# elchemista/vettore

Measured on AMD Instinct MI355X. Metric: queries/sec, flat cosine top-10, N=10000000 d=768 (achieved HBM GB/s in roofline), higher is better.
Workload: dtype f32; 1 GPU; index: :flat, metric: :cosine, d=768, N=10000000, limit=10, single query in flight; rows_per_gpu=10000000, reduce_order=sse2, processes=1

## Files before the change

vettore_amd/csrc/host/vt_search.h:

```cpp
#pragma once

namespace {

enum : unsigned { NEED_RANKS = 1, NEED_STRICT_RANKS = 2, NEED_BITS = 4, NEED_NORMS = 8, NEED_NZBITS = 16, NEED_SKETCH = 32 };
constexpr int kEscalate = -101;

bool lazy_ranks_ok(const Shard *ix, size_t limit) {
  const size_t lazy_want = std::min<size_t>(limit, ix->n) + (limit < ix->n ? 1 : 0);
  const size_t kmax = vt::scan_lds_bytes((uint32_t)ix->dim, vt::kMaxFusedK) ? (size_t)vt::kMaxFusedK : (size_t)vt::kSmallK;
  return !ix->ranks_clean && !ix->external_ranks && lazy_want <= kmax &&
         ix->unranked <= std::max<size_t>(65536, ix->n / 8);
}

constexpr size_t kPatternMinRows = 16384, kPatternMaxWant = 8 * (size_t)vt::kMaxFusedK;
bool pattern_metric(int metric) {
  return metric == VT_HAMMING || metric == VT_JACCARD;
}
bool pattern_search_applies(const Shard *ix, size_t limit) {
  return pattern_metric(ix->metric) && !ix->nz_bits.refused && ix->n >= kPatternMinRows &&
         std::min<size_t>(limit, ix->n) + 1 <= kPatternMaxWant;
}

bool shadow_metric(int metric) {
  return metric == VT_COSINE || metric == VT_INNER_PRODUCT || metric == VT_NEG_INNER_PRODUCT || metric == VT_L2 ||
// ... 269 lines not shown
  VT_HIP(vt::launch_sketch_tail(ta, c.stream));
  VT_HIP(hipStreamSynchronize(c.stream));
  if (c.hSkInfo.p[0] == 2u) {
    VT_TRY(c.ensure_part_lists((size_t)kSketchRescoreBlocks * k));
    vt::ScanArgs sa = scan_args(ix, c, d);
    set_gather(sa, gather_of(c.dSkRows.p), kSketchCandCap);
    sa.k = k;
    use_part_lists(sa, c);
    sa.batch_counts = c.dSkCount.p;
    sa.batch_cap = kSketchCandCap;
    VT_HIP(vt::launch_scan_batch(sa, kSketchRescoreBlocks, 1, c.stream));
    VT_HIP(vt::launch_select(c.dPartKeys.p, c.dPartPay.p, kSketchRescoreBlocks * k, k, 0, 0, c.dStatus.p, c.dResMapped,
                             c.dSelKeys.p, c.dSelPay.p, c.stream));
    VT_HIP(hipStreamSynchronize(c.stream));
  }
  const bool certified = c.hSkInfo.p[0] != 0u && c.hRes.p->status == 0;
  if (c.profiling) {
    float ms = 0.f;
    VT_TRY(c.span_ms(&ms));
    const uint64_t bytes = (uint64_t)vt::sketch_bytes(ix->n, d);
    c.prof.sketch_launches += 1;
    c.prof.sketch_ms += ms;
    c.prof.sketch_bytes += bytes;
    c.prof.sketch_candidates += c.hSkInfo.p[1];
    c.prof.sketch_tail_rescored += c.hSkInfo.p[0] == 1u ? 1 : 0;
    VT_TRY(c.book_scan(1, ix->n, bytes));
  }
  if (!certified) {
    c.prof.sketch_fallbacks += 1;
    return VT_OK;
  }
  std::vector<vt::Entry> entries(c.hRes.p->e, c.hRes.p->e + c.hRes.p->count);
  VT_TRY(make_hits(ix, entries, out));
  *done = true;
  return VT_OK;
}

int sketch6_search(Shard *ix, Ctx &c, const float *query, size_t limit, bool *done, vt_hits **out, int bits = 6) {
  const SketchKind &kind = sketch_kind(bits);
  const bool five = bits == 5;
  *done = false;
  const uint32_t d = (uint32_t)ix->dim, ld = ix->ld, ld8 = vt::sketch_ld8(d);
  double qq = 0.0;
  for (uint32_t i = 0; i < d; ++i) qq += (double)query[i] * (double)query[i];
  const double up = 1.0 + 0x1p-30;
  const double qn = std::sqrt(qq) * up;
  if (!(qn * ix->*kind.max_norm * up < 0x1p126)) return VT_OK;
  const uint32_t lw = vt_host::sketch6_level_words(d);
  const size_t qwords = (size_t)ld + (size_t)vt::kSketch6Levels * lw;
  const size_t chain_zeros = vt::kScanFilterSyncWords;
  const size_t total = qwords + (kind.exact_threshold ? chain_zeros : 0);
  VT_TRY(c.dQ.ensure(total));
  VT_TRY(c.hQ.ensure(total));
  if (c.hSkResid.size() < d) c.hSkResid.resize(d);
  float *hq = c.hQ.p;
  std::memcpy(hq, query, (size_t)d * sizeof(float));
  for (uint32_t i = d; i < ld; ++i) hq[i] = 0.0f;
  float t[vt::kSketch6Levels];
  double ee = 0.0;
  static_assert(vt::kSketch6Levels == vt_host::kSketch6Levels, "one number of query levels on both sides");
  vt_host::sketch6_query_levels(query, d, reinterpret_cast<uint32_t *>(hq + ld), c.hSkResid.data(), t, &ee);
  if (kind.exact_threshold) std::memset(hq + qwords, 0, chain_zeros * sizeof(float));
  uint32_t *chain_words = reinterpret_cast<uint32_t *>(c.dQ.p + qwords);
  c.qbits_kind = 0;
  c.qsrc = c.dQ.p;
  VT_HIP(hipMemcpyAsync(c.dQ.p, c.hQ.p, total * sizeof(float), hipMemcpyHostToDevice, c.stream));

  const uint32_t kp = kSketch6ListK, k = (uint32_t)limit;
  const uint32_t blocks = (uint32_t)c.num_cus * 4u, lists = blocks * kind.block_lists;
  VT_TRY(c.dSkKeys.ensure((size_t)lists * kp));
  VT_TRY(c.dSkPay.ensure((size_t)lists * kp));
  VT_TRY(c.dSkLoWords.ensure((size_t)lists * kp));
  VT_TRY(c.dSkHiWords.ensure((size_t)lists * kp));
  const uint32_t cand_cap = kind.cand_cap, rescore_blocks = kind.rescore_blocks;
  DevBuf<uint32_t> &cand_rows = c.*kind.cand_rows;
  VT_TRY(cand_rows.ensure(cand_cap));
  VT_TRY(c.dSkCount.ensure(1));
  const uint32_t thresh_blocks = vt::sketch_thresh_blocks(lists, kp);
  VT_TRY(c.dSkParts.ensure((size_t)thresh_blocks * (2 * k + 1) + 1));
  VT_TRY(c.dSkSync.ensure(4));
  VT_TRY(c.hSkInfo.ensure(4));
  VT_TRY(c.ensure_part_lists(std::max<size_t>((size_t)rescore_blocks * k, vt::kScanFilterCap)));
  uint32_t *info = c.hSkInfo.mapped();
  if (!info) return fail(VT_ERR_DEVICE, "hipHostGetDevicePointer (sketch status)");
  vt::Sketch6ScanArgs a{};
  a.img = (ix->*kind.col).buf.p;
  a.id_rank = ix->dRank.p;
  a.qimg = reinterpret_cast<const uint32_t *>(c.dQ.p + ld);
  a.n = ix->n;
  a.d = d;
  a.ld8 = ld8;
  a.metric = ix->metric;
  for (int j = 0; j < vt::kSketch6Levels; ++j) a.t[j] = t[j];
  a.qn = qn;
  a.eta = std::sqrt(ee) * up;
  a.kerr = 8.0 * d * 0x1p-24;
  {
    int64_t pos = 0, neg = 0, l1 = 0;
    const uint32_t *last = reinterpret_cast<const uint32_t *>(hq + ld) + (size_t)(vt::kSketch6Levels - 1) * lw;
    if (bits == 4) {
      a.c3 = a.w3 = 0.0;
    } else if (five) {
      vt_host::sketch5_level_bound(last, lw, t[vt::kSketch6Levels - 1], &a.c3, &a.w3);
    } else {
      vt_host::sketch6_level_sums(last, lw, &pos, &neg, &l1);
      const double t3 = 1.5 * (double)t[vt::kSketch6Levels - 1];
      a.c3 = t3 * (double)(pos + neg);
      a.w3 = t3 * (double)l1;
    }
  }
  a.k = kp;
  a.part_keys = c.dSkKeys.p;
  a.part_pay = c.dSkPay.p;
  a.lo_words = c.dSkLoWords.p;
  a.hi_words = c.dSkHiWords.p;
  VT_TRY(c.mark_begin());
  VT_HIP(kind.scan(a, blocks, c.stream));
  VT_TRY(c.mark_end());
  vt::SketchSpreadArgs ta{};
  ta.lo_words = c.dSkLoWords.p;
  ta.hi_words = c.dSkHiWords.p;
  ta.pay = c.dSkPay.p;
  ta.lists = lists;
  ta.kp = kp;
  ta.k = k;
  ta.cap = cand_cap;
  ta.parts = c.dSkParts.p;
  ta.live = c.dSkParts.p + (size_t)thresh_blocks * k;
  ta.sync = c.dSkSync.p;
  ta.rows = cand_rows.p;
  ta.count = c.dSkCount.p;
  ta.info = info;
  if (kind.exact_threshold) ta.slots = ta.live + thresh_blocks;
  VT_HIP(vt::launch_sketch_thresh(ta, c.stream));
  if (kind.exact_threshold) {
    vt::SketchRefineArgs ra{};
    ra.parts = ta.parts;
    ra.slots = ta.slots;
    ra.live = ta.live;
    ra.thresh_blocks = thresh_blocks;
    ra.k = k;
    ra.pay = c.dSkPay.p;
    ra.slots_total = lists * kp;
    ra.X = ix->dX;
    ra.stride = ld;
    ra.q = c.qsrc;
    ra.d = d;
    ra.metric = ix->metric;
    ra.order = ix->order;
    ra.kt_out = ta.slots + (size_t)thresh_blocks * k;
    VT_HIP(vt::launch_sketch_refine(ra, c.stream));
    ta.kt_word = ra.kt_out;
  }
  VT_HIP(vt::launch_sketch_collect(ta, c.stream));
  vt::ScanArgs sa = scan_args(ix, c, d);
  set_gather(sa, gather_of(cand_rows.p), cand_cap);
  sa.k = k;
  use_part_lists(sa, c);
  sa.batch_counts = c.dSkCount.p;
  sa.batch_cap = cand_cap;
  bool delivered = false;
  if (kind.exact_threshold) {
    vt::ScanArgs fa = sa;
    fa.hi_word = ta.kt_word;
    fa.surv_keys = c.dPartKeys.p;
    fa.surv_pay = c.dPartPay.p;
    fa.surv_cap = vt::kScanFilterCap;
    fa.fsync = chain_words;
    fa.out = c.dResMapped;
    fa.info = info;
    VT_HIP(vt::launch_scan_filter(fa, rescore_blocks, c.stream));
    VT_HIP(hipStreamSynchronize(c.stream));
    delivered = c.hSkInfo.p[0] == vt::kScanFilterDelivered;
  }
  if (!delivered && (!kind.exact_threshold || c.hSkInfo.p[0] == 2u)) {
    VT_HIP(vt::launch_scan_batch(sa, rescore_blocks, 1, c.stream));
    VT_HIP(vt::launch_select(c.dPartKeys.p, c.dPartPay.p, rescore_blocks * k, k, 0, 0, c.dStatus.p, c.dResMapped,
                             c.dSelKeys.p, c.dSelPay.p, c.stream));
    VT_HIP(hipStreamSynchronize(c.stream));
  }
  const bool certified = (delivered || c.hSkInfo.p[0] == 2u) && c.hRes.p->status == 0;
  if (delivered && certified) c.prof.sketch4_finished += 1;
  if (c.profiling) {
    float ms = 0.f;
    VT_TRY(c.span_ms(&ms));
    const uint64_t bytes = (uint64_t)kind.bytes(ix->n, d);
    c.prof.*kind.launches += 1;
    c.prof.*kind.ms += ms;
    c.prof.*kind.bytes_read += bytes;
    c.prof.*kind.candidates += c.hSkInfo.p[1];
    if (bits == 6) c.prof.sketch6_tail_words += c.hSkInfo.p[3] == 1u ? 1 : 0;
    VT_TRY(c.book_scan(1, ix->n, bytes));
  }
  std::atomic<uint32_t> &misses = ix->*kind.misses;
  if (!certified) {
    c.prof.*kind.fallbacks += 1;
    misses.fetch_add(1, std::memory_order_relaxed);
    return VT_OK;
  }
  misses.store(0, std::memory_order_relaxed);
  std::vector<vt::Entry> entries(c.hRes.p->e, c.hRes.p->e + c.hRes.p->count);
  VT_TRY(make_hits(ix, entries, out));
  *done = true;
  return VT_OK;
}

int sketch5_search(Shard *ix, Ctx &c, const float *query, size_t limit, bool *done, vt_hits **out) {
  return sketch6_search(ix, c, query, limit, done, out, 5);
}

int sketch4_search(Shard *ix, Ctx &c, const float *query, size_t limit, bool *done, vt_hits **out) {
  return sketch6_search(ix, c, query, limit, done, out, 4);
}

int search_ready(Shard *ix, Ctx &c, const float *query, size_t n, size_t limit, vt_hits **out, bool lone = false) {
  if (limit == 0) return empty_hits(out);
  VT_TRY(validate_vector(query, n, ix->dim));
  if (ix->n == 0) return empty_hits(out);
  if (lone && sketch4_wanted(ix, limit) && ix->sketch4.current(sketch4_elems(ix)) &&
      ix->sketch4_misses.load(std::memory_order_relaxed) < kSketch4MissLimit) {
    bool done = false;
    VT_TRY(sketch4_search(ix, c, query, limit, &done, out));
    if (done) return VT_OK;
  }
  if (lone && sketch5_wanted(ix, limit) && ix->sketch5.current(sketch5_elems(ix)) &&
      ix->sketch5_misses.load(std::memory_order_relaxed) < kSketch5MissLimit) {
    bool done = false;
    VT_TRY(sketch5_search(ix, c, query, limit, &done, out));
    if (done) return VT_OK;
  }
  if (lone && sketch6_wanted(ix, limit) && ix->sketch6.current(sketch6_elems(ix)) &&
      ix->sketch6_misses.load(std::memory_order_relaxed) < kSketch6MissLimit) {
    bool done = false;
    VT_TRY(sketch6_search(ix, c, query, limit, &done, out));
    if (done) return VT_OK;
  }
  if (lone && sketch_wanted(ix, limit) && ix->sketch.current(sketch_elems(ix))) {
    bool done = false;
    VT_TRY(sketch_search(ix, c, query, limit, &done, out));
    if (done) return VT_OK;
  }
  if (single_nominate_applies(ix, limit)) {
    std::vector<char> done(1, 0);
    vt_hits *one = nullptr;
    VT_TRY(batch_group(ix, c, query, 1, limit, &one, done, true, nullptr, nullptr));
    if (done[0]) {
      *out = one;
      return VT_OK;
    }
    delete one;
    c.prof.batch_fallbacks += 1;
  }
  const bool lazy = !ix->ranks_clean;
  const size_t lazy_want = std::min<size_t>(limit, ix->n) + (limit < ix->n ? 1 : 0);
  const bool by_pattern = pattern_search_applies(ix, limit) && !shard_stale(ix, NEED_NZBITS, limit);
  uint32_t qnz = 0;
  VT_TRY(upload_query(c, query, n, &qnz, by_pattern ? 2 : 0));
  vt::ScanArgs j = scan_args(ix, c, (uint32_t)ix->dim);
  j.q_nonzero = qnz;
  std::vector<vt::Entry> entries;
  auto best_rows = [&](size_t want) -> int {
    if (by_pattern)
      return run_hamming(c, ix->nz_bits.buf.p, c.dQbits, ix->dRank.p, ix->n, j.d, want, entries, true, ix->metric == VT_JACCARD);
    return run_scan(c, j, want, entries, true);
  };
  if (lazy) {
    VT_TRY(best_rows(lazy_want));
    const bool ambiguous = limit < ix->n && entries.size() == lazy_want &&
                           rank_key_of(entries[limit - 1].key) == rank_key_of(entries[limit].key);
    if (ambiguous) return kEscalate;
    if (entries.size() > limit) entries.resize(limit);
    for (size_t i = 0; i < entries.size();) {
      size_t e = i + 1;
      while (e < entries.size() && rank_key_of(entries[e].key) == rank_key_of(entries[i].key)) ++e;
      if (e - i > 1)
        std::sort(entries.begin() + i, entries.begin() + e,
                  [&](const vt::Entry &a, const vt::Entry &b) { return ix->ids[a.row] < ix->ids[b.row]; });
      i = e;
    }
    return make_hits(ix, entries, out);
  }
  VT_TRY(best_rows(limit));
  return make_hits(ix, entries, out);
}

int search_owner(Shard *ix, const float *query, size_t n, size_t limit, vt_hits **out) {
  const unsigned need = NEED_RANKS | NEED_NZBITS | NEED_SKETCH;
  if (shard_stale(ix, need, limit)) VT_TRY(shard_prepare(ix, need, limit));
  int st = search_ready(ix, ix->ctx, query, n, limit, out, true);
  if (st == kEscalate) {
    VT_TRY(shard_prepare(ix, NEED_STRICT_RANKS, limit));
    st = search_ready(ix, ix->ctx, query, n, limit, out, true);
  }
  return st;
}

int run_cosine_scan(Ctx &c, Shard *ix, uint32_t d, double qq, size_t want, std::vector<vt::Entry> &out) {
  const size_t kmax = vt::cosine_scan_lds_bytes(d, vt::kMaxFusedK) ? (size_t)vt::kMaxFusedK : (size_t)vt::kSmallK;
  if (vt::cosine_scan_lds_bytes(d, 1) == 0) return fail(VT_ERR_UNSUPPORTED, "prefix too long for the cosine scan kernel");
  uint64_t lo = 0;
  bool has_lo = false;
  const size_t total = std::min<size_t>(want, ix->n);
  if (out.empty() && threshold_applies(total, ix->n, (double)ix->n * vt::padded_dim(d) * 4.0, 90e-6)) {
    const uint32_t k = (uint32_t)total;
    VT_TRY(c.dKeyCol.ensure(((size_t)ix->n + 1) / 2 * 2));
    VT_TRY(c.ensure_part_lists(kThresholdListCap));
    vt::CosineScanArgs a = cosine_scan_args(ix, c, d, qq);
    a.k = 1;
    a.key_out = c.dKeyCol.p;
    uint32_t blocks = 0;
    VT_TRY(cosine_scan_all(c, a, &blocks));
    VT_TRY(threshold_rows(c, ix->n, k));
    VT_TRY(c.ensure_cand_lists(k));
    vt::CosineRerankArgs g = cosine_rerank_args(ix, c, d);
    set_gather(g, gather_of(c.dListPay.p), k);
    VT_HIP(vt::launch_cosine_rerank(g, c.stream));
    const int rc = collect_sorted_list(c, c.dCandKeys.p, c.dCandPay.p, k, out);
    if (c.profiling && rc != kRetryInternal) VT_TRY(c.book_prefix((uint64_t)ix->n * d * 4));
    if (rc != kRetryInternal) return rc;
    out.clear();
  }
  while (out.size() < total) {
    const uint32_t k = (uint32_t)std::min<size_t>(kmax, total - out.size());
    vt::CosineScanArgs a = cosine_scan_args(ix, c, d, qq);
    a.k = k;
    a.lo_key = lo;
    a.has_lo = has_lo ? 1 : 0;
    uint32_t blocks = 0;
// ... 298 lines not shown
```

vettore_amd/csrc/vt_device.h:

```cpp
#pragma once
#include <hip/hip_runtime.h>
#include <stddef.h>
#include <stdint.h>

namespace vt {

struct Payload {
  uint32_t row;
  float raw;
};
struct Entry {
  uint64_t key;
  uint32_t row;
  float raw;
};
static_assert(sizeof(Entry) == 16 && sizeof(Payload) == 8, "layout");

constexpr uint64_t kEmptyKey = ~0ull;
constexpr int kTileRows = 32;
constexpr int kWavesPerBlock = 4;
constexpr int kMaxFusedK = 256;
constexpr int kSmallK = 64;
constexpr uint32_t kRowAlign = 64;

// ... 540 lines not shown
enum { kPrepNone = 0, kPrepL2 = 1, kPrepZscore = 2, kPrepMinmax = 3 };
struct PrepareArgs {
  const float *in;
  size_t ld_in;
  float *out;
  size_t ld_out;
  uint64_t *words;
  uint32_t *first_refused;
  uint32_t n, d;
};
hipError_t launch_prepare_rows(const PrepareArgs &a, int mode, hipStream_t s);

constexpr uint32_t kSketchTileRows = 64;
constexpr uint32_t kSketchMaxDim = 32768;
__host__ __device__ inline uint32_t sketch_ld8(uint32_t d) { return (d + 127) / 128 * 128; }
__host__ __device__ inline size_t sketch_offset(uint32_t row, uint32_t chunk, uint32_t nch) {
  return ((size_t)(row / kSketchTileRows) * (nch + 1) + chunk) * 1024 + (size_t)(row % kSketchTileRows) * 16;
}
inline size_t sketch_bytes(uint32_t rows, uint32_t d) {
  const size_t tiles = ((size_t)rows + kSketchTileRows - 1) / kSketchTileRows;
  return tiles * ((size_t)sketch_ld8(d) / 16 + 1) * 1024;
}
hipError_t launch_sketch_build(const float *X, size_t stride, uint32_t n_src, uint32_t rows_img, uint32_t d, void *img,
                               unsigned long long *max_norm, hipStream_t s);
hipError_t launch_sketch_rows(const float *X, size_t stride, const uint32_t *list, uint32_t count, uint32_t rows_img, uint32_t d,
                              void *img, unsigned long long *max_norm, hipStream_t s);

struct SketchScanArgs {
  const void *img;
  const uint32_t *id_rank;
  const int8_t *qimg;
  uint32_t n, d, nch;
  int metric;
  float t1, t2;
  double qn;
  double eta;
  double kerr;
  uint32_t k;
  uint64_t *part_keys;
  Payload *part_pay;
};
size_t sketch_scan_lds_bytes(uint32_t d, uint32_t k);
hipError_t launch_sketch_scan(const SketchScanArgs &a, uint32_t blocks, hipStream_t s);

struct SketchTailArgs {
  const uint64_t *keys;
  const Payload *pay;
  uint32_t lists, kp, k, cap;
  uint32_t *rows;
  uint32_t *count;
  uint32_t *info;
  const float *X;
  size_t stride;
  const float *q;
  const uint32_t *id_rank;
  uint32_t d;
  int metric, order;
  int *status;
  ResultBlock *out;
  uint32_t ld, ss, lds_words;
};
hipError_t launch_sketch_tail(SketchTailArgs a, hipStream_t s);

struct SketchSpreadArgs {
  const uint32_t *lo_words, *hi_words;
  const Payload *pay;
  uint32_t lists, kp, k, cap;
  uint32_t *parts;
  uint32_t *live;
  uint32_t *sync;
  uint32_t *rows;
  uint32_t *count;
  uint32_t *info;
  uint32_t thresh_blocks, collect_blocks, collect_lists;
  uint32_t *slots = nullptr;
  const uint32_t *kt_word = nullptr;
};
uint32_t sketch_thresh_blocks(uint32_t lists, uint32_t kp);
hipError_t launch_sketch_thresh(SketchSpreadArgs a, hipStream_t s);
hipError_t launch_sketch_collect(SketchSpreadArgs a, hipStream_t s);

struct SketchRefineArgs {
  const uint32_t *parts, *slots, *live;
  uint32_t thresh_blocks, k;
  const Payload *pay;
  uint32_t slots_total;
  const float *X;
  size_t stride;
  const float *q;
  uint32_t d;
  int metric, order;
  uint32_t *kt_out;
  uint32_t *picked;
  uint32_t ld, ss, np4;
};
hipError_t launch_sketch_refine(SketchRefineArgs a, hipStream_t s);

constexpr int kSketch6Levels = 3;
__host__ __device__ inline uint32_t sketch6_runs(uint32_t d) { return 3 * (sketch_ld8(d) / 64) + 1; }
__host__ __device__ inline size_t sketch6_offset(uint32_t row, uint32_t run, uint32_t runs) {
  return ((size_t)(row / kSketchTileRows) * runs + run) * 1024 + (size_t)(row % kSketchTileRows) * 16;
}
inline size_t sketch6_bytes(uint32_t rows, uint32_t d) {
  const size_t tiles = ((size_t)rows + kSketchTileRows - 1) / kSketchTileRows;
  return tiles * sketch6_runs(d) * 1024;
}
hipError_t launch_sketch6_build(const float *X, size_t stride, uint32_t n_src, uint32_t rows_img, uint32_t d, void *img,
                                unsigned long long *max_norm, hipStream_t s);
hipError_t launch_sketch6_rows(const float *X, size_t stride, const uint32_t *list, uint32_t count, uint32_t rows_img, uint32_t d,
                               void *img, unsigned long long *max_norm, hipStream_t s);

struct Sketch6ScanArgs {
  const void *img;
  const uint32_t *id_rank;
  const uint32_t *qimg;
  uint32_t n, d, ld8;
  int metric;
  float t[kSketch6Levels];
  double qn, eta, kerr;
  double c3, w3;
  uint32_t k;
  uint64_t *part_keys;
  Payload *part_pay;
  uint32_t *lo_words, *hi_words;
};
size_t sketch6_scan_lds_bytes(uint32_t d, uint32_t k);
hipError_t launch_sketch6_scan(const Sketch6ScanArgs &a, uint32_t blocks, hipStream_t s);

__host__ __device__ inline uint32_t sketch5_runs(uint32_t d) { return 5 * (sketch_ld8(d) / 128) + 1; }
inline size_t sketch5_bytes(uint32_t rows, uint32_t d) {
  const size_t tiles = ((size_t)rows + kSketchTileRows - 1) / kSketchTileRows;
  return tiles * sketch5_runs(d) * 1024;
}
hipError_t launch_sketch5_build(const float *X, size_t stride, uint32_t n_src, uint32_t rows_img, uint32_t d, void *img,
                                unsigned long long *max_norm, hipStream_t s);
hipError_t launch_sketch5_rows(const float *X, size_t stride, const uint32_t *list, uint32_t count, uint32_t rows_img, uint32_t d,
                               void *img, unsigned long long *max_norm, hipStream_t s);
size_t sketch5_scan_lds_bytes(uint32_t d, uint32_t k);
hipError_t launch_sketch5_scan(const Sketch6ScanArgs &a, uint32_t blocks, hipStream_t s);

constexpr uint32_t kSketch4BlockLists = 2;
__host__ __device__ inline uint32_t sketch4_runs(uint32_t d) { return sketch_ld8(d) / 32 + 1; }
inline size_t sketch4_bytes(uint32_t rows, uint32_t d) {
  const size_t tiles = ((size_t)rows + kSketchTileRows - 1) / kSketchTileRows;
  return tiles * sketch4_runs(d) * 1024;
}
hipError_t launch_sketch4_build(const float *X, size_t stride, uint32_t n_src, uint32_t rows_img, uint32_t d, void *img,
                                unsigned long long *max_norm, hipStream_t s);
hipError_t launch_sketch4_rows(const float *X, size_t stride, const uint32_t *list, uint32_t count, uint32_t rows_img, uint32_t d,
                               void *img, unsigned long long *max_norm, hipStream_t s);
size_t sketch4_scan_lds_bytes(uint32_t d, uint32_t k);
hipError_t launch_sketch4_scan(const Sketch6ScanArgs &a, uint32_t blocks, hipStream_t s);

}
```

vettore_amd/csrc/vt_scan.cuh:

```cuda
#pragma once
#include "vt_common.cuh"

namespace vt {
namespace dev {

constexpr uint32_t kPanelChunks = 96;

struct ScanShape {
  uint32_t ld;
  uint32_t cfull;
  uint32_t tail;
  uint32_t npanel;
  uint32_t pc;
  uint32_t pc_last;
  uint32_t ss;
  uint32_t tail_base;
  uint32_t ntiles;
  uint32_t tr;
  uint32_t segs;
  uint32_t segs_last;
  uint32_t tile_floats;
  uint32_t q_global;
};

inline bool make_scan_shape(uint32_t d, uint32_t n, ScanShape *out, uint32_t tile_rows = kTileRows) {
  if (d == 0) return false;
  ScanShape p;
  p.ld = padded_dim(d);
  p.cfull = d / 8;
  p.tail = d % 8;
  const uint32_t cpr = p.ld / 8;
  uint32_t np = (cpr + kPanelChunks - 1) / kPanelChunks;
  uint32_t pc = round_up((cpr + np - 1) / np, 8);
  while (np > 1 && (np - 1) * pc >= cpr) {
    --np;
    pc = round_up((cpr + np - 1) / np, 8);
  }
  if (pc > kPanelChunks + 8) return false;
  p.npanel = np;
  p.pc = pc;
  p.pc_last = cpr - (np - 1) * pc;
  p.tail_base = pc;
  p.ss = pc + 12;
  uint32_t tr = tile_rows == 8 || tile_rows == 16 ? tile_rows : (uint32_t)kTileRows;
  while (tr < (uint32_t)kTileRows && ((p.pc * tr / 32) % kU != 0 || (p.pc_last * tr / 32) % kU != 0 ||
                                      (p.pc * tr) % 32 != 0 || (p.pc_last * tr) % 32 != 0))
    tr *= 2;
  p.tr = tr;
  p.segs = p.pc * tr / 32;
  p.segs_last = p.pc_last * tr / 32;
  p.tile_floats = 0;
  p.q_global = 0;
  p.ntiles = (n + tr - 1) / tr;
  *out = p;
  return true;
}

struct ScanDev {
  ScanArgs a;
  ScanShape p;
};

template <int OP>
__device__ __forceinline__ float elem(int op_rt, float q, float x) {
  const int op = OP >= 0 ? OP : op_rt;
  switch (op) {
    case OP_DOT: return q * x;
    case OP_L2: {
      const float t = q - x;
      return t * t;
    }
    case OP_L1:
    case OP_LINF: return fabsf(q - x);
    case OP_HAM: return ((q != 0.0f) != (x != 0.0f)) ? 1.0f : 0.0f;
    default:
      return (((q != 0.0f) != (x != 0.0f)) ? 1.0f : 0.0f) + ((x != 0.0f) ? 4096.0f : 0.0f);
  }
}

template <int OP>
__device__ __forceinline__ f32x4 elem4(int op_rt, const f32x4 q, const f32x4 x) {
  const int op = OP >= 0 ? OP : op_rt;
  switch (op) {
    case OP_DOT: return f32x4{elem<OP_DOT>(0, q.x, x.x), elem<OP_DOT>(0, q.y, x.y), elem<OP_DOT>(0, q.z, x.z), elem<OP_DOT>(0, q.w, x.w)};
    case OP_L2: return f32x4{elem<OP_L2>(0, q.x, x.x), elem<OP_L2>(0, q.y, x.y), elem<OP_L2>(0, q.z, x.z), elem<OP_L2>(0, q.w, x.w)};
    case OP_L1:
    case OP_LINF: return f32x4{elem<OP_L1>(0, q.x, x.x), elem<OP_L1>(0, q.y, x.y), elem<OP_L1>(0, q.z, x.z), elem<OP_L1>(0, q.w, x.w)};
    case OP_HAM: return f32x4{elem<OP_HAM>(0, q.x, x.x), elem<OP_HAM>(0, q.y, x.y), elem<OP_HAM>(0, q.z, x.z), elem<OP_HAM>(0, q.w, x.w)};
    default: return f32x4{elem<OP_JAC>(0, q.x, x.x), elem<OP_JAC>(0, q.y, x.y), elem<OP_JAC>(0, q.z, x.z), elem<OP_JAC>(0, q.w, x.w)};
  }
}

template <int OP>
__device__ __forceinline__ float comb(int op_rt, float a, float b) {
  const int op = OP >= 0 ? OP : op_rt;
  return op == OP_LINF ? fmaxf(a, b) : a + b;
}

template <int OP, int ORDER>
__device__ __forceinline__ float chunk_sum(int op_rt, int order_rt, float p0, float p1, float p2, float p3, int odd) {
  const int order = ORDER >= 0 ? ORDER : order_rt;
  if (order == 1) {
    const float u0 = comb<OP>(op_rt, p0, dpp_xor1(p0));
    const float u1 = comb<OP>(op_rt, p1, dpp_xor1(p1));
    const float u2 = comb<OP>(op_rt, p2, dpp_xor1(p2));
    const float u3 = comb<OP>(op_rt, p3, dpp_xor1(p3));
    const float t = comb<OP>(op_rt, odd ? u1 : u0, odd ? u3 : u2);
    return comb<OP>(op_rt, t, dpp_xor1(t));
  }
  float e;
  if (order == 2)
    e = comb<OP>(op_rt, comb<OP>(op_rt, comb<OP>(op_rt, p0, p1), p2), p3);
  else if (order == 3)
    e = comb<OP>(op_rt, comb<OP>(op_rt, p0, p2), comb<OP>(op_rt, p1, p3));
  else
    e = comb<OP>(op_rt, comb<OP>(op_rt, p0, p1), comb<OP>(op_rt, p2, p3));
  return comb<OP>(op_rt, e, dpp_xor1(e));
}

template <int OP, int ORDER>
__device__ __forceinline__ float chunk_sum1(const float (&l)[8]) {
  auto c = [](float a, float b) { return comb<OP>(0, a, b); };
  if (ORDER == 1) return c(c(c(l[0], l[4]), c(l[2], l[6])), c(c(l[1], l[5]), c(l[3], l[7])));
  if (ORDER == 2) return c(c(c(c(l[0], l[1]), l[2]), l[3]), c(c(c(l[4], l[5]), l[6]), l[7]));
  if (ORDER == 3) return c(c(c(l[0], l[2]), c(l[1], l[3])), c(c(l[4], l[6]), c(l[5], l[7])));
  return c(c(c(l[0], l[1]), c(l[2], l[3])), c(c(l[4], l[5]), c(l[6], l[7])));
}

__device__ __forceinline__ float f64_as_f32_or_nan(double v) {
  return isfinite(v) && v >= -(double)FLT_MAX && v <= (double)FLT_MAX ? (float)v : __builtin_nanf("");
}
__device__ __noinline__ static float recover_overflow(int metric, const float *q, const float *x, uint32_t d) {
  double acc = 0.0;
  switch (metric) {
    case M_L2:
    case M_L2SQ:
      for (uint32_t i = 0; i < d; ++i) {
        const double t = (double)q[i] - (double)x[i];
        acc += t * t;
      }
      if (metric == M_L2) {
        const float v = (float)sqrt(acc);
        return finite_f32(v) ? v : __builtin_nanf("");
      }
      return f64_as_f32_or_nan(acc);
    case M_COS:
    case M_IP:
    case M_NIP:
      for (uint32_t i = 0; i < d; ++i) acc += (double)q[i] * (double)x[i];
      return f64_as_f32_or_nan(metric == M_NIP ? -acc : acc);
    case M_L1:
      for (uint32_t i = 0; i < d; ++i) acc += fabs((double)q[i] - (double)x[i]);
      return f64_as_f32_or_nan(acc);
    case M_LINF:
      for (uint32_t i = 0; i < d; ++i) acc = fmax(acc, fabs((double)q[i] - (double)x[i]));
      return f64_as_f32_or_nan(acc);
    default: return __builtin_nanf("");
  }
}

__device__ __forceinline__ uint32_t filter_agent_add(uint32_t *p, uint32_t v) {
  return __hip_atomic_fetch_add(p, v, __ATOMIC_RELAXED, __HIP_MEMORY_SCOPE_AGENT);
}

__device__ __forceinline__ uint32_t filter_claim(uint32_t *counter, bool on, int lane) {
  const uint64_t act = __ballot(on);
  if (!act) return 0u;
  const int leader = __ffsll((long long)act) - 1;
  uint32_t base = 0;
  if (lane == leader) base = filter_agent_add(counter, (uint32_t)__popcll(act));
  base = (uint32_t)__shfl((int)base, leader, kWave);
  return base + (uint32_t)__popcll(act & ((1ull << lane) - 1ull));
}

__device__ __forceinline__ uint32_t *filter_stored_flag() {
  __shared__ uint32_t f_stored;
  return &f_stored;
}

__device__ __forceinline__ void filter_finish(const ScanArgs &a, uint32_t nrows, uint32_t nblocks, const uint32_t *stored) {
  __shared__ uint64_t f_keys[kScanFilterCap], f_pay[kScanFilterCap];
  __shared__ uint32_t f_last, f_n;
  const uint32_t tid = threadIdx.x;
  asm volatile("s_waitcnt vmcnt(0)" ::: "memory");
  __syncthreads();
  if (tid == 0) {
    if (*stored) {
      __builtin_amdgcn_fence(__ATOMIC_RELEASE, "agent");
      asm volatile("s_waitcnt vmcnt(0)" ::: "memory");
    }
    const uint32_t groups = nblocks < kScanFilterGroups ? nblocks : kScanFilterGroups;
    const uint32_t g = blockIdx.x % groups, members = (nblocks - g + groups - 1) / groups;
    uint32_t last = 0, n = 0;
    if (filter_agent_add(a.fsync + kScanFilterLine * (1 + g), 1u) == members - 1)
      last = filter_agent_add(a.fsync + 2, 1u) == groups - 1 ? 1u : 0u;
    if (last) {
      n = filter_agent_add(a.fsync + 0, 0u);
      const uint32_t over = __hip_atomic_fetch_or(a.fsync + 1, 0u, __ATOMIC_RELAXED, __HIP_MEMORY_SCOPE_AGENT);
      if (nrows == 0) {
        a.out->count = 0;
        last = 0;
      } else if (over || n > a.surv_cap) {
        last = 0;
      }
    }
    f_last = last;
    f_n = n;
  }
  __syncthreads();
  if (!f_last) return;
  const uint32_t n = f_n;
  for (uint32_t i = tid; i < n; i += blockDim.x) {
    f_keys[i] = __hip_atomic_load(a.surv_keys + i, __ATOMIC_RELAXED, __HIP_MEMORY_SCOPE_AGENT);
    f_pay[i] = __hip_atomic_load(reinterpret_cast<const uint64_t *>(a.surv_pay + i), __ATOMIC_RELAXED, __HIP_MEMORY_SCOPE_AGENT);
  }
  __syncthreads();
  for (uint32_t i = tid; i < n; i += blockDim.x) {
    const uint64_t key = f_keys[i];
    uint32_t pos = 0;
    for (uint32_t x = 0; x < n; ++x) {
      const uint64_t kx = f_keys[x];
      pos += (kx < key || (kx == key && x < i)) ? 1u : 0u;
    }
    if (pos < a.k) {
      const uint64_t pv = f_pay[i];
      Entry e;
      e.key = key;
      e.row = (uint32_t)pv;
      e.raw = __uint_as_float((uint32_t)(pv >> 32));
      a.out->e[pos] = e;
    }
  }
  asm volatile("s_waitcnt vmcnt(0)" ::: "memory");
  __syncthreads();
  if (tid == 0) {
    a.out->count = n < a.k ? n : a.k;
    a.out->status = atomicExch(a.status, 0);
    a.info[0] = kScanFilterDelivered;
  }
}

struct Cursor {
  uint32_t t, p, s;
  uint32_t rowi, col;
};

template <int OP, int ORDER, int CAP, bool GENERAL, bool PADDED, bool QGLOBAL = false, bool FILTER = false>
__global__ __launch_bounds__(kWavesPerBlock *kWave) void scan_topk_kernel(const ScanDev sd) {
  extern __shared__ __align__(16) float lds[];
  const ScanArgs &a = sd.a;
  const ScanShape &p = sd.p;
  const int lane = threadIdx.x & (kWave - 1);
  const int wib = __builtin_amdgcn_readfirstlane(threadIdx.x >> 6);
  const int odd = lane & 1;
  const uint32_t q_lds = QGLOBAL ? 0u : p.ld;
  float *S = lds + q_lds + wib * (p.tr * p.ss);
  unsigned char *tkbuf = reinterpret_cast<unsigned char *>(lds + q_lds + kWavesPerBlock * (p.tr * p.ss)) +
                         wib * WaveTopK<CAP>::lds_bytes();

  const float *qsrc = a.q;
  const uint32_t *gather = a.gather;
  uint32_t nrows = a.n;
  uint32_t list_base = 0;
  if (GENERAL && a.batch_counts) {
    const uint32_t b = blockIdx.y;
    const uint32_t c = a.batch_counts[b];
    nrows = c < a.batch_cap ? c : a.batch_cap;
    qsrc += (size_t)b * (a.batch_qstride ? a.batch_qstride : p.ld);
    gather += (size_t)b * (a.batch_gather_stride ? a.batch_gather_stride : a.batch_cap * a.gather_stride);
    list_base = b * gridDim.x;
  }
  if (!QGLOBAL)
    for (uint32_t i = threadIdx.x; i < p.ld; i += blockDim.x) lds[i] = qsrc[i];
  if constexpr (FILTER) {
    if (threadIdx.x == 0) *filter_stored_flag() = 0;
  }
  __syncthreads();

  const int op_rt = metric_op(a.metric);
  const uint32_t total_waves = gridDim.x * kWavesPerBlock;
  const uint32_t wave_global = blockIdx.x * kWavesPerBlock + wib;
  const uint32_t ntiles = GENERAL ? (nrows + p.tr - 1) / p.tr : p.ntiles;

  WaveTopK<CAP> tk;
  if constexpr (!FILTER) tk.init(tkbuf, a.k);
  uint32_t hi_word = 0;
  if constexpr (FILTER) hi_word = *a.hi_word;

  if (wave_global < ntiles) {
    const uint32_t last_tile = wave_global + ((ntiles - 1 - wave_global) / total_waves) * total_waves;
    const uint32_t pw0 = p.pc * 8, pw1 = p.pc_last * 8;
    const uint32_t l4 = (uint32_t)lane * 4u;
    const uint32_t ir0 = l4 / pw0, ic0 = l4 - ir0 * pw0;
    const uint32_t ir1 = l4 / pw1, ic1 = l4 - ir1 * pw1;
    const uint32_t sr0 = 256u / pw0, sc0 = 256u - sr0 * pw0;
    const uint32_t sr1 = 256u / pw1, sc1 = 256u - sr1 * pw1;
    const uint32_t lastp = p.npanel - 1;

    auto enter_panel = [&](Cursor &c) {
      const bool last = c.p == lastp;
      c.rowi = last ? ir1 : ir0;
      c.col = last ? ic1 : ic0;
    };
    auto step_lane = [&](Cursor &c) {
      const bool last = c.p == lastp;
      const uint32_t pw = last ? pw1 : pw0;
      c.rowi += last ? sr1 : sr0;
      c.col += last ? sc1 : sc0;
      if (c.col >= pw) {
        c.col -= pw;
        c.rowi += 1;
      }
    };
    uint32_t pf_idx = 0, pf_idx_prev = 0, pf_idx_next = 0;
    auto tile_index = [&](uint32_t t) -> uint32_t {
      const uint32_t g0 = t * p.tr;
      if (g0 >= nrows || g0 / p.tr != t) return 0u;
      if (!gather) return ((uint32_t)lane < p.tr && g0 + (uint32_t)lane < nrows) ? g0 + (uint32_t)lane : 0u;
      typedef const __attribute__((address_space(4))) uint32_t *cu32_p;
      cu32_p sg = (cu32_p)(uintptr_t)(gather + (size_t)g0 * a.gather_stride);
      uint32_t v = 0;
      const uint32_t left = nrows - g0;
      for (uint32_t i0 = 0; i0 < p.tr; i0 += 8) {
        uint32_t sv[8];
#pragma unroll
        for (uint32_t j = 0; j < 8; ++j) {
          const uint32_t i = i0 + j < left ? i0 + j : left - 1;
          sv[j] = sg[(size_t)i * a.gather_stride];
        }
#pragma unroll
        for (uint32_t j = 0; j < 8; ++j) v = (uint32_t)lane == i0 + j ? sv[j] : v;
      }
      return v;
    };
    auto advance = [&](Cursor &c) {
      const uint32_t nseg = c.p == lastp ? p.segs_last : p.segs;
      c.s += 1;
      if (c.s == nseg) {
        c.s = 0;
        c.p += 1;
        if (c.p == p.npanel) {
          c.p = 0;
          c.t += total_waves;
          if (GENERAL) {
            pf_idx_prev = pf_idx;
            pf_idx = pf_idx_next;
            pf_idx_next = tile_index(c.t + total_waves);
          }
        }
        enter_panel(c);
      } else {
        step_lane(c);
      }
    };
    auto load_at = [&](const Cursor &c) -> f32x4 {
      const uint32_t t = c.t < last_tile ? c.t : last_tile;
      const uint32_t colf = c.p * pw0 + c.col;
      if (!GENERAL) {
        const float *base = a.X + (size_t)t * p.tile_floats;
        return __builtin_nontemporal_load(reinterpret_cast<const f32x4 *>(base + (c.rowi * (uint32_t)a.stride + colf)));
      }
      (void)t;
      const uint32_t src = (uint32_t)__shfl((int)pf_idx, (int)c.rowi, kWave);
      return __builtin_nontemporal_load(reinterpret_cast<const f32x4 *>(a.X + (size_t)src * a.stride + colf));
    };

    Cursor pf;
    pf.t = wave_global;
    pf.p = 0;
    pf.s = 0;
    enter_panel(pf);
    if (GENERAL) {
      pf_idx = tile_index(wave_global);
      pf_idx_next = tile_index(wave_global + total_waves);
    }
    f32x4 buf[kU];
#pragma unroll
    for (int u = 0; u < kU; ++u) {
      buf[u] = load_at(pf);
      advance(pf);
    }

    for (uint32_t t = wave_global; t < ntiles; t += total_waves) {
      const uint32_t grow = t * p.tr + lane;
      const bool row_valid = (uint32_t)lane < p.tr && grow < nrows;
      uint32_t src_row = grow;
      if (GENERAL && gather) src_row = pf.t == t ? pf_idx : pf_idx_prev;
      uint32_t my_rank = src_row;
      if (row_valid && a.id_rank) my_rank = a.id_rank[src_row];

      float acc = 0.0f;
      uint32_t jac_ham = 0, jac_xnz = 0;
// ... 176 lines not shown
```

Baseline: 1437 queries/s.

## Fuse sketch candidate collection into exact rescore filter for dot metrics

Adds a sketch4 rescore kernel that reads the per-list sketch hi-words and payloads directly and rescores the qualifying rows, instead of first running a separate collect kernel and then a gather-based scan filter. The collect launch is deferred, so it runs only if the filtered path fails to deliver. The goal is to remove one kernel launch and the intermediate candidate-list write and read on the hot path. In exchange it adds a new kernel with per-block staging, its own overflow/fail signalling through the sync words, and a templated filter_finish decision hook.

```diff
diff --git a/vettore_amd/csrc/host/vt_search.h b/vettore_amd/csrc/host/vt_search.h
--- a/vettore_amd/csrc/host/vt_search.h
+++ b/vettore_amd/csrc/host/vt_search.h
@@ -445,7 +445,10 @@
     VT_HIP(vt::launch_sketch_refine(ra, c.stream));
     ta.kt_word = ra.kt_out;
   }
-  VT_HIP(vt::launch_sketch_collect(ta, c.stream));
+  const bool dot_metric = ix->metric == VT_COSINE || ix->metric == VT_INNER_PRODUCT || ix->metric == VT_NEG_INNER_PRODUCT;
+  const bool from_lists = kind.exact_threshold && dot_metric && k <= (uint32_t)vt::kSmallK && ta.kt_word &&
+                          vt::sketch4_rescore_lds_bytes(d, kp) != 0;
+  if (!from_lists) VT_HIP(vt::launch_sketch_collect(ta, c.stream));
   vt::ScanArgs sa = scan_args(ix, c, d);
   set_gather(sa, gather_of(cand_rows.p), cand_cap);
   sa.k = k;
@@ -462,11 +465,24 @@
     fa.fsync = chain_words;
     fa.out = c.dResMapped;
     fa.info = info;
-    VT_HIP(vt::launch_scan_filter(fa, rescore_blocks, c.stream));
+    if (from_lists) {
+      vt::Sketch4RescoreArgs ra{};
+      ra.s = fa;
+      ra.s.gather = nullptr;
+      ra.s.batch_counts = nullptr;
+      ra.hi_words = ta.hi_words;
+      ra.pay = ta.pay;
+      ra.kp = kp;
+      ra.cap = cand_cap;
+      VT_HIP(vt::launch_sketch4_rescore(ra, blocks, c.stream));
+    } else {
+      VT_HIP(vt::launch_scan_filter(fa, rescore_blocks, c.stream));
+    }
     VT_HIP(hipStreamSynchronize(c.stream));
     delivered = c.hSkInfo.p[0] == vt::kScanFilterDelivered;
   }
   if (!delivered && (!kind.exact_threshold || c.hSkInfo.p[0] == 2u)) {
+    if (from_lists) VT_HIP(vt::launch_sketch_collect(ta, c.stream));
     VT_HIP(vt::launch_scan_batch(sa, rescore_blocks, 1, c.stream));
     VT_HIP(vt::launch_select(c.dPartKeys.p, c.dPartPay.p, rescore_blocks * k, k, 0, 0, c.dStatus.p, c.dResMapped,
                              c.dSelKeys.p, c.dSelPay.p, c.stream));
diff --git a/vettore_amd/csrc/vt_device.h b/vettore_amd/csrc/vt_device.h
--- a/vettore_amd/csrc/vt_device.h
+++ b/vettore_amd/csrc/vt_device.h
@@ -716,4 +716,14 @@
 size_t sketch4_scan_lds_bytes(uint32_t d, uint32_t k);
 hipError_t launch_sketch4_scan(const Sketch6ScanArgs &a, uint32_t blocks, hipStream_t s);
 
-}
+struct Sketch4RescoreArgs {
+  ScanArgs s;
+  const uint32_t *hi_words;
+  const Payload *pay;
+  uint32_t kp, cap;
+  uint32_t ld, ss;
+};
+size_t sketch4_rescore_lds_bytes(uint32_t d, uint32_t kp);
+hipError_t launch_sketch4_rescore(Sketch4RescoreArgs a, uint32_t blocks, hipStream_t s);
+
+}
diff --git a/vettore_amd/csrc/vt_scan.cuh b/vettore_amd/csrc/vt_scan.cuh
--- a/vettore_amd/csrc/vt_scan.cuh
+++ b/vettore_amd/csrc/vt_scan.cuh
@@ -1,5 +1,7 @@
 #pragma once
 #include "vt_common.cuh"
+
+#include <type_traits>
 
 namespace vt {
 namespace dev {
@@ -178,7 +180,10 @@
   return &f_stored;
 }
 
-__device__ __forceinline__ void filter_finish(const ScanArgs &a, uint32_t nrows, uint32_t nblocks, const uint32_t *stored) {
+struct FilterAsCollected {};
+template <typename Decide>
+__device__ __forceinline__ void filter_finish(const ScanArgs &a, uint32_t nrows, uint32_t nblocks, const uint32_t *stored,
+                                              Decide decide) {
   __shared__ uint64_t f_keys[kScanFilterCap], f_pay[kScanFilterCap];
   __shared__ uint32_t f_last, f_n;
   const uint32_t tid = threadIdx.x;
@@ -194,15 +199,19 @@
     uint32_t last = 0, n = 0;
     if (filter_agent_add(a.fsync + kScanFilterLine * (1 + g), 1u) == members - 1)
       last = filter_agent_add(a.fsync + 2, 1u) == groups - 1 ? 1u : 0u;
-    if (last) {
-      n = filter_agent_add(a.fsync + 0, 0u);
-      const uint32_t over = __hip_atomic_fetch_or(a.fsync + 1, 0u, __ATOMIC_RELAXED, __HIP_MEMORY_SCOPE_AGENT);
-      if (nrows == 0) {
-        a.out->count = 0;
-        last = 0;
-      } else if (over || n > a.surv_cap) {
-        last = 0;
-      }
+    if constexpr (std::is_same<Decide, FilterAsCollected>::value) {
+      if (last) {
+        n = filter_agent_add(a.fsync + 0, 0u);
+        const uint32_t over = __hip_atomic_fetch_or(a.fsync + 1, 0u, __ATOMIC_RELAXED, __HIP_MEMORY_SCOPE_AGENT);
+        if (nrows == 0) {
+          a.out->count = 0;
+          last = 0;
+        } else if (over || n > a.surv_cap) {
+          last = 0;
+        }
+      }
+    } else {
+      if (last) last = decide(&n) ? 1u : 0u;
     }
     f_last = last;
     f_n = n;
@@ -238,6 +247,10 @@
     a.out->status = atomicExch(a.status, 0);
     a.info[0] = kScanFilterDelivered;
   }
+}
+
+__device__ __forceinline__ void filter_finish(const ScanArgs &a, uint32_t nrows, uint32_t nblocks, const uint32_t *stored) {
+  filter_finish(a, nrows, nblocks, stored, FilterAsCollected{});
 }
 
 struct Cursor {
diff --git a/vettore_amd/csrc/vt_sketch4_rescore.hip b/vettore_amd/csrc/vt_sketch4_rescore.hip
--- /dev/null
+++ b/vettore_amd/csrc/vt_sketch4_rescore.hip
@@ -0,0 +1,240 @@
+#include "vt_scan.cuh"
+
+namespace vt {
+namespace dev {
+
+constexpr uint32_t kRoundRows = 6;
+constexpr uint32_t kStaticSegs = 3;
+constexpr uint32_t kRoundLoads = kRoundRows * kStaticSegs;
+constexpr uint32_t kLongLoads = 12;
+constexpr uint32_t kFailBit = 2u;
+
+__host__ __device__ inline uint32_t rescore_round_rows(uint32_t nseg) {
+  const uint32_t r = (nseg <= kStaticSegs ? kRoundLoads : kLongLoads) / nseg;
+  return r < kRoundRows ? r : kRoundRows;
+}
+
+template <int ORDER, int NSEG>
+__global__ __launch_bounds__(kWavesPerBlock *kWave, 4) void sketch4_rescore_kernel(const Sketch4RescoreArgs a) {
+  extern __shared__ __align__(16) float lds[];
+  __shared__ uint32_t s_n;
+  const ScanArgs &f = a.s;
+  const uint32_t tid = threadIdx.x;
+  const int lane = tid & (kWave - 1);
+  const int wib = __builtin_amdgcn_readfirstlane(tid >> 6);
+  const int odd = lane & 1;
+  constexpr uint32_t kLoads = NSEG ? kRoundRows * NSEG : kLongLoads;
+  const uint32_t nseg = NSEG ? (uint32_t)NSEG : (a.ld + 255u) / 256u, rr = rescore_round_rows(nseg);
+  float *S = lds + a.ld + (uint32_t)wib * (rr * a.ss);
+  uint32_t *stage = reinterpret_cast<uint32_t *>(lds + a.ld + kWavesPerBlock * (rr * a.ss));
+  uint32_t *lcnt = stage + kSketch4BlockLists * a.kp;
+
+  static_assert(kSketch4BlockLists * kSmallK <= kWavesPerBlock * kWave, "a thread per slot");
+  const uint32_t slots = kSketch4BlockLists * a.kp, first = blockIdx.x * slots;
+  const uint32_t h = tid < slots ? a.hi_words[first + tid] : 0xffffffffu;
+  const uint32_t row = tid < slots ? a.pay[first + tid].row : 0u;
+  const uint32_t kt = *f.hi_word;
+  for (uint32_t i = tid; i < a.ld; i += blockDim.x) lds[i] = f.q[i];
+  if (tid < kSketch4BlockLists) lcnt[tid] = 0;
+  if (tid == 0) {
+    s_n = 0;
+    *filter_stored_flag() = 0;
+  }
+  __syncthreads();
+
+  {
+    const uint32_t i = tid;
+    const bool cand = h != 0xffffffffu && h <= kt;
+    const uint64_t act = __ballot(cand);
+    if (act) {
+      const int leader = __ffsll((long long)act) - 1;
+      uint32_t base = 0;
+      if (lane == leader) base = atomicAdd(&s_n, (uint32_t)__popcll(act));
+      base = (uint32_t)__shfl((int)base, leader, kWave);
+      if (cand) {
+        stage[base + (uint32_t)__popcll(act & ((1ull << lane) - 1ull))] = row;
+        atomicAdd(&lcnt[i / a.kp], 1u);
+      }
+    }
+  }
+  __syncthreads();
+  const uint32_t n = s_n;
+  const uint32_t groups = gridDim.x < kScanFilterGroups ? gridDim.x : kScanFilterGroups;
+  if (tid == 0 && n) filter_agent_add(f.fsync + kScanFilterLine * (1 + blockIdx.x % groups) + 1, n);
+  if (tid < kSketch4BlockLists && lcnt[tid] == a.kp)
+    __hip_atomic_fetch_or(f.fsync + 1, kFailBit, __ATOMIC_RELAXED, __HIP_MEMORY_SCOPE_AGENT);
+
+  const uint32_t cfull = f.d / 8, tail = f.d % 8, tail_base = a.ss - 12;
+  const uint32_t nw = n > (uint32_t)wib ? (n - (uint32_t)wib + kWavesPerBlock - 1) / kWavesPerBlock : 0u;
+  const uint32_t l4 = (uint32_t)lane * 4u;
+  const int order = ORDER >= 0 ? ORDER : f.order;
+  for (uint32_t i0 = 0; i0 < nw; i0 += rr) {
+    const uint32_t left = nw - i0 < rr ? nw - i0 : rr;
+    const bool chain = (uint32_t)lane < left;
+    const uint32_t my_row = stage[(uint32_t)wib + kWavesPerBlock * (i0 + (chain ? (uint32_t)lane : 0u))];
+    uint32_t my_rank = my_row;
+    if (chain && f.id_rank) my_rank = f.id_rank[my_row];
+
+    f32x4 x[kLoads];
+    {
+      uint32_t r = 0, s = 0;
+#pragma unroll
+      for (uint32_t j = 0; j < kLoads; ++j) {
+        const uint32_t ru = r < left ? r : 0u;
+        const uint32_t src = (uint32_t)__builtin_amdgcn_readlane((int)my_row, (int)ru);
+        const uint32_t col = s * 256u + l4, colc = col < a.ld ? col : a.ld - 4u;
+        x[j] = __builtin_nontemporal_load(reinterpret_cast<const f32x4 *>(f.X + (size_t)src * f.stride + colc));
+        if (++s == nseg) {
+          s = 0;
+          r = r + 1 < rr ? r + 1 : r;
+        }
+      }
+    }
+    {
+      uint32_t r = 0, s = 0;
+      bool live = true;
+#pragma unroll
+      for (uint32_t j = 0; j < kLoads; ++j) {
+        const uint32_t col = s * 256u + l4, colc = col < a.ld ? col : a.ld - 4u;
+        const f32x4 qv = *reinterpret_cast<const f32x4 *>(lds + colc);
+        const f32x4 pr = elem4<OP_DOT>(OP_DOT, qv, x[j]);
+        const float sum = chunk_sum<OP_DOT, ORDER>(OP_DOT, order, pr.x, pr.y, pr.z, pr.w, odd);
+        const uint32_t ch = col >> 3;
+        float *Srow = S + r * a.ss;
+        if (live && r < left && col < a.ld) {
+          if (ch < cfull) {
+            if (!odd) Srow[ch] = sum;
+          } else if (ch == cfull) {
+            *reinterpret_cast<f32x4 *>(Srow + tail_base + odd * 4) = pr;
+          }
+        }
+        if (++s == nseg) {
+          s = 0;
+          if (r + 1 < rr) r = r + 1;
+          else live = false;
+        }
+      }
+    }
+    wave_lds_fence();
+
+    float acc = 0.0f;
+    if (chain) {
+      const float *Sr = S + (uint32_t)lane * a.ss;
+      uint32_t c = 0;
+      constexpr uint32_t kBatch = 12;
+      for (; c + 4 * kBatch <= cfull; c += 4 * kBatch) {
+        f32x4 v[kBatch];
+#pragma unroll
+        for (uint32_t j = 0; j < kBatch; ++j) v[j] = *reinterpret_cast<const f32x4 *>(Sr + c + 4 * j);
+#pragma unroll
+        for (uint32_t j = 0; j < kBatch; ++j) {
+          acc = acc + v[j].x;
+          acc = acc + v[j].y;
+          acc = acc + v[j].z;
+          acc = acc + v[j].w;
+        }
+      }
+      for (; c + 4 <= cfull; c += 4) {
+        const f32x4 v = *reinterpret_cast<const f32x4 *>(Sr + c);
+        acc = acc + v.x;
+        acc = acc + v.y;
+        acc = acc + v.z;
+        acc = acc + v.w;
+      }
+      for (; c < cfull; ++c) acc = acc + Sr[c];
+      for (uint32_t j = 0; j < tail; ++j) acc = acc + Sr[tail_base + j];
+    }
+    wave_lds_fence();
+    const int metric = f.metric;
+    float raw = metric == M_NIP ? -acc : acc;
+    bool valid = chain;
+    if (valid && !finite_f32(raw)) {
+      const float rec = recover_overflow(metric, f.q, f.X + (size_t)my_row * f.stride, f.d);
+      if (rec == rec) {
+        raw = rec;
+      } else {
+        atomicMax(f.status, kErrOverflow);
+        valid = false;
+      }
+    }
+    float rank = raw;
+    if (metric == M_COS) rank = 1.0f - raw;
+    else if (metric == M_IP) rank = -raw;
+    const uint64_t key = ((uint64_t)orderable(rank) << 32) | my_rank;
+    const bool keep = valid && (uint32_t)(key >> 32) <= kt;
+    const uint32_t pos = filter_claim(f.fsync + 0, keep, lane);
+    if (keep) {
+      if (pos < f.surv_cap) {
+        *filter_stored_flag() = 1;
+        f.surv_keys[pos] = key;
+        Payload pv;
+        pv.row = my_row;
+        pv.raw = raw;
+        f.surv_pay[pos] = pv;
+      } else {
+        __hip_atomic_fetch_or(f.fsync + 1, 1u, __ATOMIC_RELAXED, __HIP_MEMORY_SCOPE_AGENT);
+      }
+    }
+  }
+
+  filter_finish(f, 1u, gridDim.x, filter_stored_flag(), [&](uint32_t *nsurv) {
+    const uint32_t ns = __hip_atomic_load(f.fsync + 0, __ATOMIC_RELAXED, __HIP_MEMORY_SCOPE_AGENT);
+    const uint32_t over = __hip_atomic_load(f.fsync + 1, __ATOMIC_RELAXED, __HIP_MEMORY_SCOPE_AGENT);
+    uint32_t part[kScanFilterGroups];
+#pragma unroll
+    for (uint32_t g = 0; g < kScanFilterGroups; ++g)
+      part[g] = g < groups ? __hip_atomic_load(f.fsync + kScanFilterLine * (1 + g) + 1, __ATOMIC_RELAXED, __HIP_MEMORY_SCOPE_AGENT) : 0u;
+    uint32_t total = 0;
+#pragma unroll
+    for (uint32_t g = 0; g < kScanFilterGroups; ++g) total += part[g];
+    const bool ok = !(over & kFailBit) && total <= a.cap;
+    f.info[0] = ok ? 2u : 0u;
+    f.info[1] = total;
+    f.info[2] = kt;
+    f.info[3] = 1u;
+    *nsurv = ns;
+    return ok && !over && ns <= f.surv_cap;
+  });
+}
+
+template <int ORDER, int NSEG>
+static hipError_t launch_rescore_t(const Sketch4RescoreArgs &a, uint32_t blocks, size_t lds, hipStream_t s) {
+  hipLaunchKernelGGL((sketch4_rescore_kernel<ORDER, NSEG>), dim3(blocks), dim3(kWavesPerBlock * kWave), lds, s, a);
+  return hipGetLastError();
+}
+template <int ORDER>
+static hipError_t launch_rescore_segs(const Sketch4RescoreArgs &a, uint32_t blocks, size_t lds, hipStream_t s) {
+  static_assert(kStaticSegs == 3, "an instantiation per static segment count");
+  const uint32_t nseg = (a.ld + 255u) / 256u;
+  if (nseg == 1) return launch_rescore_t<ORDER, 1>(a, blocks, lds, s);
+  if (nseg == 2) return launch_rescore_t<ORDER, 2>(a, blocks, lds, s);
+  if (nseg == 3) return launch_rescore_t<ORDER, 3>(a, blocks, lds, s);
+  return launch_rescore_t<ORDER, 0>(a, blocks, lds, s);
+}
+}
+
+using namespace dev;
+
+size_t sketch4_rescore_lds_bytes(uint32_t d, uint32_t kp) {
+  if (d == 0 || kp == 0 || kp > (uint32_t)kSmallK) return 0;
+  const uint32_t ld = padded_dim(d), nseg = (ld + 255u) / 256u;
+  if (nseg > kLongLoads) return 0;
+  const size_t ss = ld / 8 + 12;
+  const size_t bytes = ((size_t)ld + (size_t)kWavesPerBlock * rescore_round_rows(nseg) * ss + (size_t)kSketch4BlockLists * kp + 4) * 4;
+  return bytes <= kMaxLds / 4 - 18 * 1024 ? bytes : 0;
+}
+
+hipError_t launch_sketch4_rescore(Sketch4RescoreArgs a, uint32_t blocks, hipStream_t s) {
+  const ScanArgs &f = a.s;
+  const size_t lds = sketch4_rescore_lds_bytes(f.d, a.kp);
+  if (!lds || blocks == 0 || f.k == 0 || f.k > (uint32_t)kSmallK || f.k > a.kp || metric_op(f.metric) != OP_DOT || f.has_lo ||
+      f.stride < padded_dim(f.d) || !f.X || !f.q || !a.hi_words || !a.pay || !f.hi_word || !f.surv_keys || !f.surv_pay ||
+      f.surv_cap == 0 || f.surv_cap > kScanFilterCap || !f.fsync || !f.out || !f.info || !f.status)
+    return hipErrorInvalidValue;
+  a.ld = padded_dim(f.d);
+  a.ss = a.ld / 8 + 12;
+  if (f.order == kDefaultReduceOrder) return launch_rescore_segs<kDefaultReduceOrder>(a, blocks, lds, s);
+  return launch_rescore_segs<-1>(a, blocks, lds, s);
+}
+
+}
```

After: 1456 queries/s, median of 6. 1.01x the previous value.
